# dronefreak/CABiNet

Hardware: AMD Instinct MI355X
Metric: 1024x1024 images/sec fwd+bwd (CABiNet-MobileNetV3-Large) (higher is better)
Workload: dtype f32; 1 GPU; BASELINE configs[2]: CABiNet-MobileNetV3-Large, 8x3x1024x1024 synthetic 8-class per GPU, fwd + 2x OhemCE + bwd + grad all-reduce + SGD step, HIP CAB/FFM kernels, fp32, random-init (model seed 0, gamma=0.5); per_gpu_batch=8, global_batch=8, n_classes=8, parallelism=dp1, miopen_find_mode=FAST

## Files before the change

### cabinet_amd/csrc/conv3x3_s2.hip

```cpp
#include "common.hpp"
#include "slab_sum.hpp"

namespace cabinet {

struct C3Shape {
    int B, H, W, Ho, Wo;
};

static C3Shape c3_shape(int B, int H, int W) { return C3Shape{B, H, W, (H - 1) / 2 + 1, (W - 1) / 2 + 1}; }

constexpr int CW_C = 64;
constexpr int CW_TW = 32;
constexpr int CW_IW = 2 * CW_TW + 1;
constexpr int CW_XP = 3 * CW_IW;
constexpr int CW_DLD = CW_TW + 1;
constexpr int CW_SLAB = CW_C * CW_C * 9;
constexpr int CW_TARGET_WG = 512;
constexpr int CW_MIN_ROWS = 4;

struct C3Plan {
    int tiles_x, strips, rows_per;
};

static C3Plan cw_plan(const C3Shape& s) {
    C3Plan p;
    p.tiles_x = ceil_div(s.Wo, CW_TW);
    const long per = (long)s.B * p.tiles_x;
    long strips = CW_TARGET_WG / per;
    const int cap = ceil_div(s.Ho, CW_MIN_ROWS);
    if (strips > cap) strips = cap;
    if (strips < 1) strips = 1;
    p.rows_per = ceil_div(s.Ho, (int)strips);
    p.strips = ceil_div(s.Ho, p.rows_per);
    return p;
}

__global__ __launch_bounds__(256, 2) void conv3x3s2_wgrad64_kernel(const float* __restrict__ dy, const float* __restrict__ x,
                                                                 C3Shape s, int tiles_x, int strips, int rows_per,
                                                                 float* __restrict__ slabs) {
    extern __shared__ __attribute__((aligned(16))) float smem[];
    float* xs = smem;
    float* dys = xs + CW_C * CW_XP;
    const int tid = threadIdx.x, wave = tid >> 6, lane = tid & 63, li = lane & 31, h = lane >> 5;
    int bi = blockIdx.x;
    const int tx = bi % tiles_x;
    bi /= tiles_x;
    const int strip = bi % strips, b = bi / strips;
    const int oy_begin = strip * rows_per, oy_end = min(s.Ho, oy_begin + rows_per);
    const int ox0 = tx * CW_TW, ix0 = 2 * ox0 - 1;
    const int ch = wave & 1, cj = wave >> 1;

    f32x16 acc[9];
#pragma unroll
    for (int t = 0; t < 9; ++t)
#pragma unroll
        for (int r = 0; r < 16; ++r) acc[t][r] = 0.f;

    const float* xb = x + (size_t)b * CW_C * s.H * s.W;
    const float* dyb = dy + (size_t)b * CW_C * s.Ho * s.Wo;
    const float* arow = dys + (32 * ch + li) * CW_DLD + h;
    const float* brow = xs + (32 * cj + li) * CW_XP + 2 * h;
    for (int oy = oy_begin; oy < oy_end; ++oy) {
        const int iy0 = 2 * oy - 1;
        __syncthreads();
        for (int i = tid; i < CW_C * CW_XP; i += 256) {
            const int ci = i / CW_XP, r = i - ci * CW_XP, yy = r / CW_IW, xx = r - yy * CW_IW;
            const int iy = iy0 + yy, ix = ix0 + xx;
            xs[i] = (iy >= 0 && iy < s.H && ix >= 0 && ix < s.W) ? xb[((size_t)ci * s.H + iy) * s.W + ix] : 0.f;
        }
        for (int i = tid; i < CW_C * CW_TW; i += 256) {
            const int co = i >> 5, c = i & 31, ox = ox0 + c;
            dys[co * CW_DLD + c] = ox < s.Wo ? dyb[((size_t)co * s.Ho + oy) * s.Wo + ox] : 0.f;
        }
        __syncthreads();
#pragma unroll
        for (int c0 = 0; c0 < CW_TW; c0 += 2) {
            const float a = arow[c0];
#pragma unroll
            for (int ky = 0; ky < 3; ++ky)
#pragma unroll
                for (int kx = 0; kx < 3; ++kx)
                    acc[3 * ky + kx] = mfma32(a, brow[ky * CW_IW + 2 * c0 + kx], acc[3 * ky + kx]);
        }
    }
    float* slab = slabs + (size_t)blockIdx.x * CW_SLAB;
#pragma unroll
    for (int r = 0; r < 16; ++r) {
        const int co = 32 * ch + acc_row(r) + 4 * h, ci = 32 * cj + li;
        float* p = slab + (co * CW_C + ci) * 9;
#pragma unroll
        for (int t = 0; t < 9; ++t) p[t] = acc[t][r];
    }
}

constexpr int CF_CI = 3, CF_CO = 16, CF_KK = CF_CI * 9;
constexpr int CF_TH = 4, CF_TW = 32;
constexpr int CF_IH = 2 * CF_TH + 1, CF_IW = 2 * CF_TW + 1;
constexpr int CF_PATCH = CF_CI * CF_IH * CF_IW;
constexpr int CF_DLD = CF_TH * CF_TW + 1;
constexpr int CF_SLAB = CF_CO * CF_KK;

__global__ __launch_bounds__(256) void conv3x3s2_wgrad_3_16_kernel(const float* __restrict__ dy, const float* __restrict__ x,
                                                                  C3Shape s, int tiles_x, float* __restrict__ slabs) {
    __shared__ __attribute__((aligned(16))) float dys[32 * CF_DLD];
    __shared__ float xs[CF_PATCH];
    __shared__ float red[4][CF_CO][32];
    const int tid = threadIdx.x, wave = tid >> 6, lane = tid & 63, li = lane & 31, h = lane >> 5;
    const int strips_y = (s.Ho + CF_TH - 1) / CF_TH;
    const int b = blockIdx.x / strips_y, oy0 = (blockIdx.x - b * strips_y) * CF_TH;
    const int kk = li < CF_KK ? li : 0;
    const int ko = ((kk / 9) * CF_IH + (kk % 9) / 3) * CF_IW + kk % 3;
    f32x16 acc;
#pragma unroll
    for (int r = 0; r < 16; ++r) acc[r] = 0.f;
    for (int i = tid; i < 16 * CF_DLD; i += 256) dys[16 * CF_DLD + i] = 0.f;
    const float* xb = x + (size_t)b * CF_CI * s.H * s.W;
    const float* dyb = dy + (size_t)b * CF_CO * s.Ho * s.Wo;
    const int iy0 = 2 * oy0 - 1;
    for (int t = 0; t < tiles_x; ++t) {
        const int ox0 = t * CF_TW, ix0 = 2 * ox0 - 1;
        __syncthreads();
        for (int i = tid; i < CF_PATCH; i += 256) {
            const int ci = i / (CF_IH * CF_IW), r = i - ci * CF_IH * CF_IW, yy = r / CF_IW, xx = r - yy * CF_IW;
            const int iy = iy0 + yy, ix = ix0 + xx;
            xs[i] = (iy >= 0 && iy < s.H && ix >= 0 && ix < s.W) ? xb[((size_t)ci * s.H + iy) * s.W + ix] : 0.f;
        }
        for (int i = tid; i < CF_CO * CF_TH * CF_TW; i += 256) {
            const int co = i / (CF_TH * CF_TW), p = i - co * (CF_TH * CF_TW), r = p / CF_TW, c = p - r * CF_TW;
            const int oy = oy0 + r, ox = ox0 + c;
            dys[co * CF_DLD + p] = (oy < s.Ho && ox < s.Wo) ? dyb[((size_t)co * s.Ho + oy) * s.Wo + ox] : 0.f;
        }
        __syncthreads();
        const float* drow = dys + li * CF_DLD + 32 * wave + h;
        const float* prow = xs + ko + 2 * wave * CF_IW + 2 * h;
#pragma unroll
        for (int c0 = 0; c0 < 32; c0 += 2) acc = mfma32(drow[c0], prow[2 * c0], acc);
    }
#pragma unroll
    for (int r = 0; r < 16; ++r) {
        const int co = acc_row(r) + 4 * h;
        if (co < CF_CO) red[wave][co][li] = acc[r];
    }
    __syncthreads();
    float* slab = slabs + (size_t)blockIdx.x * CF_SLAB;
    for (int i = tid; i < CF_SLAB; i += 256) {
        const int co = i / CF_KK, k = i - co * CF_KK;
        slab[i] = ((red[0][co][k] + red[1][co][k]) + red[2][co][k]) + red[3][co][k];
    }
}

typedef float f32x4v __attribute__((ext_vector_type(4)));
__device__ __forceinline__ f32x4v mfma16(float a, float b, f32x4v c) { return __builtin_amdgcn_mfma_f32_16x16x4f32(a, b, c, 0, 0, 0); }

constexpr int CD_NT = 64;
constexpr int CD_RP = 80;
constexpr int CD_SLOTS = 3;
constexpr int CD_CP = CD_SLOTS * CD_RP;
constexpr int CD_PR = CW_C / 4;

__device__ __forceinline__ float cd_ld(const float* base, unsigned byte_off) {
    return *reinterpret_cast<const float*>(reinterpret_cast<const char*>(base) + byte_off);
}

__host__ __device__ constexpr int cd_par(int k) { return k == 1 ? 0 : 1; }
__host__ __device__ constexpr int cd_shift(int k) { return k == 0 ? 1 : 0; }

__global__ __launch_bounds__(256, 2) void conv3x3s2_dgrad64_kernel(const float* __restrict__ dy, const float* __restrict__ w,
                                                                 C3Shape s, int tiles_n, int strips, int rows_per,
                                                                 float* __restrict__ dx) {
    __shared__ __attribute__((aligned(16))) float dys[CW_C * CD_CP];
    const int tid = threadIdx.x, wave = __builtin_amdgcn_readfirstlane(tid >> 6), lane = tid & 63, lc = lane & 15, lk = lane >> 4;
    int bi = blockIdx.x;
    const int tn = bi % tiles_n;
    bi /= tiles_n;
    const int strip = bi % strips, b = bi / strips;
    const int m_begin = strip * rows_per, m_end = min(s.Ho, m_begin + rows_per);
    const int n0 = tn * CD_NT;
    const int ci0 = 16 * wave;

    float wr[9][16];
#pragma unroll
    for (int t = 0; t < 9; ++t)
#pragma unroll
        for (int ks = 0; ks < 16; ++ks) wr[t][ks] = w[((4 * ks + lk) * CW_C + ci0 + lc) * 9 + t];

    const float* dyb = dy + (size_t)b * CW_C * s.Ho * s.Wo;
    float* dxb = dx + ((size_t)b * CW_C + ci0 + 4 * lk) * s.H * s.W;
    const float* brow = dys + lk * CD_CP + lc;
    const bool pair_ok = (s.W & 1) == 0;
    const unsigned colo = (unsigned)min(n0 + lane, s.Wo - 1) * 4u;
    const bool col_ok = n0 + lane < s.Wo, halo_ok = n0 + CD_NT < s.Wo;
    float pp[CD_PR + 1];
    auto request = [&](int r) {
        const int oy = min(r, s.Ho - 1);
#pragma unroll
        for (int j = 0; j < CD_PR; ++j) pp[j] = cd_ld(dyb + ((size_t)(CD_PR * wave + j) * s.Ho + oy) * s.Wo, colo);
        int te = tid;
        asm volatile("" : "+v"(te));
        pp[CD_PR] = dyb[((size_t)min(te, CW_C - 1) * s.Ho + oy) * s.Wo + min(n0 + CD_NT, s.Wo - 1)];
    };
    auto commit = [&](int r, int slot) {
        const bool row_ok = r < s.Ho;
        float* d = dys + slot * CD_RP;
#pragma unroll
        for (int j = 0; j < CD_PR; ++j) d[(CD_PR * wave + j) * CD_CP + lane] = (row_ok && col_ok) ? pp[j] : 0.f;
        if (tid < CW_C) d[tid * CD_CP + CD_NT] = (row_ok && halo_ok) ? pp[CD_PR] : 0.f;
    };
    request(m_begin);
    commit(m_begin, 0);
    request(m_begin + 1);
    int s0 = 0;
    for (int m = m_begin; m < m_end; ++m) {
        const int s1 = s0 == CD_SLOTS - 1 ? 0 : s0 + 1;
        commit(m + 1, s1);
        __syncthreads();
        if (m + 1 < m_end) request(m + 2);
        const float* bp0 = brow + s0 * CD_RP;
        const float* bp1 = brow + s1 * CD_RP;
        s0 = s1;
#pragma unroll 1
        for (int ng = 0; ng < CD_NT / 16 && n0 + 16 * ng < s.Wo; ++ng) {
            f32x4v acc[2][2];
#pragma unroll
            for (int i = 0; i < 2; ++i)
#pragma unroll
                for (int j = 0; j < 2; ++j) acc[i][j] = f32x4v{0.f, 0.f, 0.f, 0.f};
            float bv[2][8];
            auto read_half = [&](int g, float* v) {
                const int t = g / 2;
                const float* bt = (cd_shift(t / 3) ? bp1 : bp0) + 16 * ng + cd_shift(t % 3);
#pragma unroll
                for (int i = 0; i < 8; ++i) v[i] = bt[4 * (8 * (g % 2) + i) * CD_CP];
            };
            read_half(0, bv[0]);
            f32x4v p0, p1;
#pragma unroll
            for (int g = 0; g < 18; ++g) {
                const int t = g / 2, k8 = 8 * (g % 2);
                if (g + 1 < 18) read_half(g + 1, bv[(g + 1) & 1]);
                if (g % 2 == 0) p0 = p1 = f32x4v{0.f, 0.f, 0.f, 0.f};
#pragma unroll
                for (int i = 0; i < 8; i += 2) {
                    p0 = mfma16(wr[t][k8 + i], bv[g & 1][i], p0);
                    p1 = mfma16(wr[t][k8 + i + 1], bv[g & 1][i + 1], p1);
                }
                if (g % 2 == 1) acc[cd_par(t / 3)][cd_par(t % 3)] += p0 + p1;
                __builtin_amdgcn_sched_barrier(0);
            }
            const int ix = 2 * (n0 + 16 * ng + lc);
#pragma unroll
            for (int rp = 0; rp < 2; ++rp) {
                const int iy = 2 * m + rp;
                if (iy < s.H && ix < s.W) {
#pragma unroll
                    for (int r = 0; r < 4; ++r) {
                        float* p = dxb + ((size_t)r * s.H + iy) * s.W + ix;
                        if (pair_ok) {
                            *reinterpret_cast<f32x2*>(p) = f32x2{acc[rp][0][r], acc[rp][1][r]};
                        } else {
                            p[0] = acc[rp][0][r];
                            if (ix + 1 < s.W) p[1] = acc[rp][1][r];
                        }
                    }
                }
            }
        }
    }
}

bool conv3x3s2_supported(int Ci, int Co) { return (Ci == CW_C && Co == CW_C) || (Ci == CF_CI && Co == CF_CO); }

static C3Plan cd_plan(const C3Shape& s) {
    C3Plan p;
    p.tiles_x = ceil_div(s.Wo, CD_NT);
    const long per = (long)s.B * p.tiles_x;
    long strips = CW_TARGET_WG / per;
    if (strips > s.Ho) strips = s.Ho;
    if (strips < 1) strips = 1;
    p.rows_per = ceil_div(s.Ho, (int)strips);
    p.strips = ceil_div(s.Ho, p.rows_per);
    return p;
}

long long conv3x3s2_dgrad_workgroups(int B, int H, int W) {
    const C3Shape s = c3_shape(B, H, W);
    const long long per = (long long)B * ceil_div(s.Wo, CD_NT);
    if (per > (1ll << 30)) return per;
    const C3Plan p = cd_plan(s);
    return per * p.strips;
}

hipError_t conv3x3s2_dgrad_run(const float* dy, const float* w, int B, int H, int W, float* dx, hipStream_t stream) {
    const C3Shape s = c3_shape(B, H, W);
    const C3Plan p = cd_plan(s);
    hipLaunchKernelGGL(conv3x3s2_dgrad64_kernel, dim3(B * p.tiles_x * p.strips), dim3(256), 0, stream, dy, w, s, p.tiles_x,
                       p.strips, p.rows_per, dx);
    return hipGetLastError();
}

long long conv3x3s2_wgrad_slabs(int B, int Ci, int H, int W) {
    const C3Shape s = c3_shape(B, H, W);
    if (Ci == CF_CI) return (long long)B * ceil_div(s.Ho, CF_TH);
    const long long tiles_x = ceil_div(s.Wo, CW_TW);
    if ((long long)B * tiles_x > (1ll << 30)) return (long long)B * tiles_x;
    const C3Plan p = cw_plan(s);
    return (long long)B * p.tiles_x * p.strips;
}

size_t conv3x3s2_wgrad_workspace(int B, int Ci, int H, int W) {
    return align_up((size_t)conv3x3s2_wgrad_slabs(B, Ci, H, W) * (Ci == CF_CI ? CF_SLAB : CW_SLAB) * sizeof(float), 256);
}

hipError_t conv3x3s2_wgrad_run(const float* dy, const float* x, int B, int Ci, int H, int W, float* dw, void* ws,
                               hipStream_t stream) {
    const C3Shape s = c3_shape(B, H, W);
    float* slabs = static_cast<float*>(ws);
    const int nslab = (int)conv3x3s2_wgrad_slabs(B, Ci, H, W);
    if (Ci == CF_CI) {
        hipLaunchKernelGGL(conv3x3s2_wgrad_3_16_kernel, dim3(nslab), dim3(256), 0, stream, dy, x, s, ceil_div(s.Wo, CF_TW),
                           slabs);
    } else {
        const C3Plan p = cw_plan(s);
        const size_t lds = (size_t)(CW_C * CW_XP + CW_C * CW_DLD) * sizeof(float);
        static lds_attr_mask mask{0};
        if (hipError_t e = ensure_dynamic_lds(reinterpret_cast<const void*>(conv3x3s2_wgrad64_kernel), lds, mask); e != hipSuccess)
            return e;
        hipLaunchKernelGGL(conv3x3s2_wgrad64_kernel, dim3(nslab), dim3(256), lds, stream, dy, x, s, p.tiles_x, p.strips,
                           p.rows_per, slabs);
    }
    hipError_t e = hipGetLastError();
    if (e != hipSuccess) return e;
    slab_sum_launch(slabs, nslab, Ci == CF_CI ? CF_SLAB : CW_SLAB, dw, stream);
    return hipGetLastError();
}

}
```

### cabinet_amd/functional.py

```python

from __future__ import annotations

import ctypes as _ct

import torch
import torch.nn.functional as F

from . import _lib


def _ptr(t):
    return t.data_ptr() if t is not None else None


def _stream_handle(device):
    return torch.cuda.current_stream(device).cuda_stream


def _workspace(nbytes, device):
    if nbytes == 0:
        return None, 0
    ws = torch.empty(nbytes, dtype=torch.uint8, device=device)
    return ws, nbytes

# ... 1347 lines not shown
        with torch.cuda.device(dev):
            rc = lib.cabinet_se_act_bwd_dx(_ptr(g), _ptr(z), _ptr(mean), _ptr(invstd), _ptr(bn_w), _ptr(bn_b), _ptr(gate), _ptr(ds_p),
                                           _ptr(coef), B, C, P, fn_ctx.act, _ptr(dz), stream)
        _lib.check(rc, "cabinet_se_act_bwd_dx")
        return dz, dweight, dbias, None, None, dw1, db1, dw2, db2, None, None, None, None


def se_tail(z, bn, se, act=None):
    if not z.is_cuda:
        raise RuntimeError("se_tail: device tensors only")
    if act not in _ACT_CODES:
        raise RuntimeError(f"se_tail: unknown activation {act!r}")
    fc1, fc2 = se.fc[0], se.fc[2]
    training, momentum = _bn_step(bn)
    return _SeTail.apply(z, bn.weight, bn.bias, bn.running_mean, bn.running_var, fc1.weight, fc1.bias, fc2.weight, fc2.bias,
                         _ACT_CODES[act], training, momentum, bn.eps)




class _BnActDwConv(torch.autograd.Function):
    @staticmethod
    @torch.amp.custom_fwd(device_type="cuda", cast_inputs=torch.float32)
    def forward(fn_ctx, z, bn_w, bn_b, run_mean, run_var, conv_w, act, stride, training, momentum, eps):
        lib = _lib.load()
        z, bn_w, bn_b, cw = _f32c(z), _f32c(bn_w), _f32c(bn_b), _f32c(conv_w)
        B, C, H, W = z.shape
        K = cw.shape[-1]
        Ho, Wo = (H + 2 * (K // 2) - K) // stride + 1, (W + 2 * (K // 2) - K) // stride + 1
        y = torch.empty((B, C, Ho, Wo), dtype=torch.float32, device=z.device)
        mean = torch.empty(C, dtype=torch.float32, device=z.device)
        invstd = torch.empty(C, dtype=torch.float32, device=z.device)
        ws, nbytes = _workspace(lib.cabinet_bn_dwconv_fwd_workspace_bytes(B, C, H, W), z.device)
        with torch.cuda.device(z.device):
            rc = lib.cabinet_bn_dwconv_fwd(_ptr(z), _ptr(bn_w), _ptr(bn_b), _ptr(run_mean), _ptr(run_var), _ptr(cw), B, C,
                                           H, W, K, stride, act, int(training), float(momentum), float(eps), _ptr(y),
                                           _ptr(mean), _ptr(invstd), _ptr(ws), nbytes, _stream_handle(z.device))
        _lib.check(rc, "cabinet_bn_dwconv_fwd")
        fn_ctx.save_for_backward(z, bn_w, bn_b, cw, mean, invstd)
        fn_ctx.meta = (act, stride, bool(training))
        return y

    @staticmethod
    @torch.amp.custom_bwd(device_type="cuda")
    def backward(fn_ctx, g):
        lib = _lib.load()
        z, bn_w, bn_b, cw, mean, invstd = fn_ctx.saved_tensors
        act, stride, training = fn_ctx.meta
        g = _f32c(g)
        B, C, H, W = z.shape
        K = cw.shape[-1]
        dz, dbw, dbb, dcw = torch.empty_like(z), torch.empty_like(bn_w), torch.empty_like(bn_b), torch.empty_like(cw)
        ws, nbytes = _workspace(lib.cabinet_bn_dwconv_bwd_workspace_bytes(B, C, H, W, K, stride), z.device)
        with torch.cuda.device(z.device):
            rc = lib.cabinet_bn_dwconv_bwd(_ptr(g), _ptr(z), _ptr(bn_w), _ptr(bn_b), _ptr(mean), _ptr(invstd), _ptr(cw), B,
                                           C, H, W, K, stride, act, int(training), _ptr(dz), _ptr(dbw), _ptr(dbb),
                                           _ptr(dcw), _ptr(ws), nbytes, _stream_handle(z.device))
        _lib.check(rc, "cabinet_bn_dwconv_bwd")
        return dz, dbw, dbb, None, None, dcw, None, None, None, None, None


def bn_act_dwconv(z, bn, act, conv):
    if not z.is_cuda:
        raise RuntimeError("bn_act_dwconv: device tensors only")
    if act not in _ACT_CODES:
        raise RuntimeError(f"bn_act_dwconv: unknown activation {act!r}")
    training, momentum = _bn_step(bn)
    return _BnActDwConv.apply(z, bn.weight, bn.bias, bn.running_mean, bn.running_var, conv.weight, _ACT_CODES[act],
                              conv.stride[0], training, momentum, bn.eps)




def stem_conv_supported(conv):
    return (conv.in_channels == 3 and conv.out_channels == 64 and conv.kernel_size == (7, 7) and conv.stride == (2, 2)
            and conv.padding == (3, 3) and conv.dilation == (1, 1) and conv.groups == 1 and conv.bias is None
            and conv.padding_mode == "zeros")


class _StemConv(torch.autograd.Function):
    @staticmethod
    @torch.amp.custom_fwd(device_type="cuda", cast_inputs=torch.float32)
    def forward(fn_ctx, x, weight):
        lib = _lib.load()
        x, w = _f32c(x), _f32c(weight)
        B, _, H, W = x.shape
        y = torch.empty((B, 64, (H - 1) // 2 + 1, (W - 1) // 2 + 1), dtype=torch.float32, device=x.device)
        with torch.cuda.device(x.device):
            rc = lib.cabinet_stem_conv_fwd(_ptr(x), _ptr(w), B, H, W, _ptr(y), _stream_handle(x.device))
        _lib.check(rc, "cabinet_stem_conv_fwd")
        fn_ctx.save_for_backward(x, w)
        return y

    @staticmethod
    @torch.amp.custom_bwd(device_type="cuda")
    def backward(fn_ctx, g):
        lib = _lib.load()
        x, w = fn_ctx.saved_tensors
        g = _f32c(g)
        B, _, H, W = x.shape
        dx = None
        if fn_ctx.needs_input_grad[0]:
            dx = torch.ops.aten.convolution_backward(g, x, w, None, [2, 2], [3, 3], [1, 1], False, [0, 0], 1,
                                                     [True, False, False])[0]
        dw = torch.empty_like(w)
        ws, nbytes = _workspace(lib.cabinet_stem_conv_wrw_workspace_bytes(B, H, W), x.device)
        with torch.cuda.device(x.device):
            rc = lib.cabinet_stem_conv_wrw(_ptr(g), _ptr(x), B, H, W, _ptr(dw), _ptr(ws), nbytes,
                                           _stream_handle(x.device))
        _lib.check(rc, "cabinet_stem_conv_wrw")
        return dx, dw


def stem_conv(x, conv):
    if not x.is_cuda:
        raise RuntimeError("stem_conv: device tensors only")
    return _StemConv.apply(x, conv.weight)


STEM_BN_FUSED = _os.environ.get("CABINET_STEM_BN_FUSED", "1") != "0"


class _StemConvBnRelu(torch.autograd.Function):

    @staticmethod
    @torch.amp.custom_fwd(device_type="cuda", cast_inputs=torch.float32)
    def forward(fn_ctx, x, weight, bn_weight, bn_bias, run_mean, run_var, training, momentum, eps):
        lib = _lib.load()
        x, w, bn_weight, bn_bias = _f32c(x), _f32c(weight), _f32c(bn_weight), _f32c(bn_bias)
        B, _, H, W = x.shape
        z = torch.empty((B, 64, (H - 1) // 2 + 1, (W - 1) // 2 + 1), dtype=torch.float32, device=x.device)
        y = torch.empty_like(z)
        mean = torch.empty(64, dtype=torch.float32, device=x.device)
        invstd = torch.empty(64, dtype=torch.float32, device=x.device)
        P = z.shape[2] * z.shape[3]
        with torch.cuda.device(x.device):
            rc = lib.cabinet_stem_conv_fwd(_ptr(x), _ptr(w), B, H, W, _ptr(z), _stream_handle(x.device))
            _lib.check(rc, "cabinet_stem_conv_fwd")
            ws, nbytes = _workspace(lib.cabinet_bn_act_workspace_bytes(B, 64, P), x.device)
            rc = lib.cabinet_bn_act_fwd(_ptr(z), _ptr(bn_weight), _ptr(bn_bias), _ptr(run_mean), _ptr(run_var), None, B, 64, P,
                                        _ACT_CODES["relu"], int(training), float(momentum), float(eps), _ptr(y), _ptr(mean),
                                        _ptr(invstd), _ptr(ws), nbytes, _stream_handle(x.device))
            _lib.check(rc, "cabinet_bn_act_fwd")
        fn_ctx.save_for_backward(x, z, w, bn_weight, bn_bias, mean, invstd)
        fn_ctx.training = bool(training)
        return y

    @staticmethod
    @torch.amp.custom_bwd(device_type="cuda")
    def backward(fn_ctx, g):
        lib = _lib.load()
        x, z, w, bn_weight, bn_bias, mean, invstd = fn_ctx.saved_tensors
        g = _f32c(g)
        B, _, H, W = x.shape
        dw, dgam, dbet = torch.empty_like(w), torch.empty_like(bn_weight), torch.empty_like(bn_bias)
        ws, nbytes = _workspace(lib.cabinet_stem_conv_bn_bwd_workspace_bytes(B, H, W), x.device)
        with torch.cuda.device(x.device):
            rc = lib.cabinet_stem_conv_bn_bwd(_ptr(g), _ptr(z), _ptr(x), _ptr(bn_weight), _ptr(bn_bias), _ptr(mean), _ptr(invstd),
                                              B, H, W, int(fn_ctx.training), _ptr(dw), _ptr(dgam), _ptr(dbet), _ptr(ws), nbytes,
                                              _stream_handle(x.device))
        _lib.check(rc, "cabinet_stem_conv_bn_bwd")
        return None, dw, dgam, dbet, None, None, None, None, None


def stem_conv_bn_relu(x, conv, bn):
    if not x.is_cuda:
        raise RuntimeError("stem_conv_bn_relu: device tensors only")
    if x.requires_grad:
        raise RuntimeError("stem_conv_bn_relu: the image gets no gradient here; use bn_act(stem_conv(...))")
    training, momentum = _bn_step(bn)
    return _StemConvBnRelu.apply(x, conv.weight, bn.weight, bn.bias, bn.running_mean, bn.running_var, training, momentum, bn.eps)




def pwconv_supported(conv, x):
    if not (conv.kernel_size == (1, 1) and conv.stride == (1, 1) and conv.padding == (0, 0) and conv.groups == 1
            and conv.bias is None and conv.dilation == (1, 1)):
        return False
    P = x.shape[2] * x.shape[3]
    return (P >= 65536 and conv.in_channels <= 96 and conv.out_channels <= 96
            and bool(_lib.load().cabinet_pwconv_supported(conv.in_channels, conv.out_channels, P)))


class _PwConv(torch.autograd.Function):
    @staticmethod
    @torch.amp.custom_fwd(device_type="cuda", cast_inputs=torch.float32)
    def forward(fn_ctx, x, weight):
        lib = _lib.load()
        x = _f32c(x)
        Co, Ci = weight.shape[0], weight.shape[1]
        w2 = _f32c(weight).view(Co, Ci)
        B, P = x.shape[0], x.shape[2] * x.shape[3]
        y = torch.empty((B, Co) + tuple(x.shape[2:]), dtype=torch.float32, device=x.device)
        with torch.cuda.device(x.device):
            rc = lib.cabinet_pwconv_fwd(_ptr(x), _ptr(w2), B, Ci, Co, P, _ptr(y), _stream_handle(x.device))
        _lib.check(rc, "cabinet_pwconv_fwd")
        fn_ctx.save_for_backward(x, w2)
        fn_ctx.w_shape = weight.shape
        return y

    @staticmethod
    @torch.amp.custom_bwd(device_type="cuda")
    def backward(fn_ctx, g):
        lib = _lib.load()
        x, w2 = fn_ctx.saved_tensors
        g = _f32c(g)
        Co, Ci = w2.shape
        B, P = x.shape[0], x.shape[2] * x.shape[3]
        dx = torch.empty_like(x) if fn_ctx.needs_input_grad[0] else None
        dw = torch.empty_like(w2) if fn_ctx.needs_input_grad[1] else None
        ws, nbytes = _workspace(lib.cabinet_pwconv_bwd_workspace_bytes(B, Ci, Co, P), x.device)
        with torch.cuda.device(x.device):
            rc = lib.cabinet_pwconv_bwd(_ptr(g), _ptr(x), _ptr(w2), B, Ci, Co, P, _ptr(dx), _ptr(dw), _ptr(ws), nbytes,
                                        _stream_handle(x.device))
        _lib.check(rc, "cabinet_pwconv_bwd")
        return dx, (dw.view(fn_ctx.w_shape) if dw is not None else None)


def pwconv(x, conv):
    if not x.is_cuda:
        raise RuntimeError("pwconv: device tensors only")
    return _PwConv.apply(x, conv.weight)




PWCONV_WIDE_ENABLED = _os.environ.get("CABINET_PWCONV_WIDE", "1") != "0"


def pwconv_wide_supported(conv, x):
    if not (PWCONV_WIDE_ENABLED and isinstance(conv, torch.nn.Conv2d) and x.is_cuda and x.dim() == 4):
        return False
    if not (conv.kernel_size == (1, 1) and conv.stride == (1, 1) and conv.padding == (0, 0) and conv.groups == 1
            and conv.bias is None and conv.dilation == (1, 1)):
        return False
    if not (torch.is_grad_enabled() and conv.weight.requires_grad) or torch.is_autocast_enabled():
        return False
    if x.dtype != torch.float32 or conv.weight.dtype != torch.float32 or x.shape[0] < 1 or x.shape[2] * x.shape[3] < 1:
        return False
    return bool(_lib.load().cabinet_pwconv_wide_supported(conv.in_channels, conv.out_channels, x.shape[2] * x.shape[3]))


class _PwConvWide(torch.autograd.Function):

    @staticmethod
    def forward(fn_ctx, x, weight):
        x = x.contiguous()
        y = F.conv2d(x, weight)
        fn_ctx.save_for_backward(x, weight)
        return y

    @staticmethod
    def backward(fn_ctx, g):
        x, w = fn_ctx.saved_tensors
        g = g.contiguous()
        dx = None
        if fn_ctx.needs_input_grad[0]:
            dx = torch.ops.aten.convolution_backward(g, x, w, None, [1, 1], [0, 0], [1, 1], False, [0, 0], 1,
                                                     [True, False, False])[0]
        dw = None
        if fn_ctx.needs_input_grad[1]:
            lib = _lib.load()
            xc, gc = _f32c(x), _f32c(g)
            Co, Ci = w.shape[0], w.shape[1]
            B, P = xc.shape[0], xc.shape[2] * xc.shape[3]
            dw = torch.empty((Co, Ci, 1, 1), dtype=torch.float32, device=x.device)
            ws, nbytes = _workspace(lib.cabinet_pwconv_wide_wgrad_workspace_bytes(B, Ci, Co, P), x.device)
            with torch.cuda.device(x.device):
                rc = lib.cabinet_pwconv_wide_wgrad(_ptr(gc), _ptr(xc), B, Ci, Co, P, _ptr(dw), _ptr(ws), nbytes,
                                                   _stream_handle(x.device))
            _lib.check(rc, "cabinet_pwconv_wide_wgrad")
        return dx, dw


def pwconv_wide(x, conv):
    if not x.is_cuda:
        raise RuntimeError("pwconv_wide: device tensors only")
    return _PwConvWide.apply(x, conv.weight)




CONV3X3S2_ENABLED = _os.environ.get("CABINET_CONV3X3S2", "1") != "0"


def conv3x3s2_supported(conv, x):
    if not (CONV3X3S2_ENABLED and isinstance(conv, torch.nn.Conv2d) and x.is_cuda and x.dim() == 4):
        return False
    if not (conv.kernel_size == (3, 3) and conv.stride == (2, 2) and conv.padding == (1, 1) and conv.groups == 1
            and conv.bias is None and conv.dilation == (1, 1) and conv.padding_mode == "zeros"):
        return False
    if not (torch.is_grad_enabled() and conv.weight.requires_grad) or torch.is_autocast_enabled():
        return False
    if x.dtype != torch.float32 or conv.weight.dtype != torch.float32 or x.shape[0] < 1 or x.shape[2] * x.shape[3] < 1:
        return False
    return x.shape[1] == conv.in_channels and bool(_lib.load().cabinet_conv3x3s2_supported(conv.in_channels, conv.out_channels))


def _conv3x3s2_native_wgrad(Ci, B, H):
    return Ci == 3 and B * (((H - 1) // 2 + 1 + 3) // 4) >= 1024


class _Conv3x3S2(torch.autograd.Function):

    @staticmethod
    def forward(fn_ctx, x, weight):
        x = x.contiguous()
        y = F.conv2d(x, weight, None, 2, 1)
        fn_ctx.save_for_backward(x, weight)
        return y

    @staticmethod
    def backward(fn_ctx, g):
        x, w = fn_ctx.saved_tensors
        g = g.contiguous()
        lib = _lib.load()
        xc, gc = _f32c(x), _f32c(g)
        Co, Ci = w.shape[0], w.shape[1]
        B, H, W = xc.shape[0], xc.shape[2], xc.shape[3]
        cb = torch.ops.aten.convolution_backward
        dx = None
        if fn_ctx.needs_input_grad[0] and Ci == 64:
            dx = torch.empty_like(xc)
            with torch.cuda.device(x.device):
                rc = lib.cabinet_conv3x3s2_dgrad(_ptr(gc), _ptr(_f32c(w)), B, Ci, Co, H, W, _ptr(dx), _stream_handle(x.device))
            _lib.check(rc, "cabinet_conv3x3s2_dgrad")
        elif fn_ctx.needs_input_grad[0]:
            dx = cb(g, x, w, None, [2, 2], [1, 1], [1, 1], False, [0, 0], 1, [True, False, False])[0]
        dw = None
        if fn_ctx.needs_input_grad[1] and _conv3x3s2_native_wgrad(Ci, B, H):
            dw = torch.empty((Co, Ci, 3, 3), dtype=torch.float32, device=x.device)
            ws, nbytes = _workspace(lib.cabinet_conv3x3s2_wgrad_workspace_bytes(B, Ci, Co, H, W), x.device)
            with torch.cuda.device(x.device):
                rc = lib.cabinet_conv3x3s2_wgrad(_ptr(gc), _ptr(xc), B, Ci, Co, H, W, _ptr(dw), _ptr(ws), nbytes,
                                                 _stream_handle(x.device))
            _lib.check(rc, "cabinet_conv3x3s2_wgrad")
        elif fn_ctx.needs_input_grad[1]:
            dw = cb(g, x, w, None, [2, 2], [1, 1], [1, 1], False, [0, 0], 1, [False, True, False])[1]
        return dx, dw


class Conv2dS2(torch.nn.Conv2d):

    def _conv_forward(self, input, weight, bias):
        if bias is None and conv3x3s2_supported(self, input):
            return _Conv3x3S2.apply(input, weight)
        return super()._conv_forward(input, weight, bias)




def eval_chip_accum_supported(logits, chip_size, flip=False):
    if not (logits.is_cuda and logits.dim() == 4 and _lib.available()):
        return False
    _, C, hl, wl = logits.shape
    return bool(_lib.load().cabinet_eval_chip_accum_supported(C, hl, wl, int(chip_size[0]), int(chip_size[1]), int(bool(flip))))


def eval_chip_accum(dst, logits, logits_flipped, chip_size, origin, rcp_y=None, rcp_x=None):
    lib = _lib.load()
    if not (dst.is_cuda and dst.dtype == torch.float32 and dst.is_contiguous()):
        raise RuntimeError("eval_chip_accum: dst must be a dense fp32 device tensor")
    a = _f32c(logits)
    b = _f32c(logits_flipped) if logits_flipped is not None else None
    if b is not None and b.shape != a.shape:
        raise RuntimeError("eval_chip_accum: the flipped chip's logits must have the shape of the chip's")
    N, C, hl, wl = a.shape
    if dst.shape[:2] != (N, C):
        raise RuntimeError(f"eval_chip_accum: dst {tuple(dst.shape)} does not match logits {tuple(a.shape)}")
    FH, FW = dst.shape[2:]
    ry = _f32c(rcp_y) if rcp_y is not None else None
    rx = _f32c(rcp_x) if rcp_x is not None else None
    if (ry is not None and ry.numel() != FH) or (rx is not None and rx.numel() != FW):
        raise RuntimeError("eval_chip_accum: rcp_y / rcp_x must have one entry per row / column of dst")
    dev = dst.device
    with torch.cuda.device(dev):
        rc = lib.cabinet_eval_chip_accum(_ptr(a), _ptr(b), N, C, hl, wl, int(chip_size[0]), int(chip_size[1]), _ptr(dst), FH, FW,
                                         int(origin[0]), int(origin[1]), _ptr(ry), _ptr(rx), _stream_handle(dev))
    _lib.check(rc, "cabinet_eval_chip_accum")
    return dst


def eval_scale_merge_supported(total):
    return bool(total.is_cuda and total.dim() == 4 and _lib.available() and total.shape[0] * total.shape[1] <= 65535
                and total.shape[2] <= 65535)


def eval_scale_merge(total, prob, crop=None):
    lib = _lib.load()
    if not (total.is_cuda and total.dtype == torch.float32 and total.is_contiguous()):
        raise RuntimeError("eval_scale_merge: total must be a dense fp32 device tensor")
    prob = _f32c(prob)
    N, C, H, W = total.shape
    if prob.shape[:2] != (N, C):
        raise RuntimeError(f"eval_scale_merge: prob {tuple(prob.shape)} does not match total {tuple(total.shape)}")
    FH, FW = prob.shape[2:]
    hst, hed, wst, wed = crop if crop is not None else (0, FH, 0, FW)
    dev = total.device
    with torch.cuda.device(dev):
        rc = lib.cabinet_eval_scale_merge(_ptr(prob), N, C, FH, FW, int(hst), int(hed), int(wst), int(wed), _ptr(total), H, W,
                                          _stream_handle(dev))
    _lib.check(rc, "cabinet_eval_scale_merge")
    return total


def eval_argmax_hist_supported(total):
    return bool(total.is_cuda and total.dim() == 4 and _lib.available() and total.shape[1] <= 32)


def eval_argmax_hist(total, labels, hist, ignore_label, want_pred=False):
    lib = _lib.load()
    if not (total.is_cuda and total.dtype == torch.float32 and total.is_contiguous()):
        raise RuntimeError("eval_argmax_hist: total must be a dense fp32 device tensor")
    N, C, H, W = total.shape
    if labels.dtype != torch.int64 or tuple(labels.shape) != (N, H, W) or labels.device != total.device:
        raise RuntimeError("eval_argmax_hist: labels must be (N, H, W) int64 on total's device")
    if hist.dtype != torch.int64 or tuple(hist.shape) != (C, C) or not hist.is_contiguous() or hist.device != total.device:
        raise RuntimeError("eval_argmax_hist: hist must be a dense (C, C) int64 tensor on total's device")
    labels = _aligned(labels)
    pred = torch.empty((N, H, W), dtype=torch.uint8, device=total.device) if want_pred else None
    dev = total.device
    with torch.cuda.device(dev):
        rc = lib.cabinet_eval_argmax_hist(_ptr(total), _ptr(labels), N, C, H, W, int(ignore_label), _ptr(hist), _ptr(pred),
                                          _stream_handle(dev))
    _lib.check(rc, "cabinet_eval_argmax_hist")
    return pred




def _u8_out(out, shape, device, what):
    if out is None:
        return torch.empty(shape, dtype=torch.uint8, device=device)
    if not (out.dtype == torch.uint8 and out.device == device and tuple(out.shape) == tuple(shape) and out.is_contiguous()):
        raise RuntimeError(f"{what}: out must be a dense uint8 tensor of shape {tuple(shape)} on the input's device")
    return out


def predict_up_argmax_supported(logits, size):
    if not (logits.is_cuda and logits.dim() == 4 and _lib.available()):
        return False
    N, C, hl, wl = logits.shape
    return bool(N <= 65535 and _lib.load().cabinet_predict_up_argmax_supported(C, hl, wl, int(size[0]), int(size[1])))


def predict_up_argmax(logits, size, out=None):
    lib = _lib.load()
    if not (logits.is_cuda and logits.dim() == 4):
        raise RuntimeError("predict_up_argmax: logits must be a (N, C, h, w) device tensor")
    a = _f32c(logits)
    N, C, hl, wl = a.shape
    H, W = int(size[0]), int(size[1])
    labels = _u8_out(out, (N, H, W), a.device, "predict_up_argmax")
    dev = a.device
    with torch.cuda.device(dev):
        rc = lib.cabinet_predict_up_argmax(_ptr(a), N, C, hl, wl, H, W, _ptr(labels), _stream_handle(dev))
    _lib.check(rc, "cabinet_predict_up_argmax")
    return labels


def predict_argmax_supported(total):
    return bool(total.is_cuda and total.dim() == 4 and _lib.available() and total.shape[1] <= 32 and total.shape[0] <= 65535)


def predict_argmax(total, out=None):
    lib = _lib.load()
    if not (total.is_cuda and total.dim() == 4):
        raise RuntimeError("predict_argmax: total must be a (N, C, H, W) device tensor")
    t = _f32c(total)
    N, C, H, W = t.shape
    labels = _u8_out(out, (N, H, W), t.device, "predict_argmax")
    dev = t.device
    with torch.cuda.device(dev):
        rc = lib.cabinet_predict_argmax(_ptr(t), N, C, H, W, _ptr(labels), _stream_handle(dev))
    _lib.check(rc, "cabinet_predict_argmax")
    return labels


def predict_render(labels, image, palette, mean=(0.485, 0.456, 0.406), std=(0.229, 0.224, 0.225), alpha=0.6,
                   want_input=True, want_overlay=True, out=None):
    lib = _lib.load()
    if not (labels.is_cuda and labels.dtype == torch.uint8 and labels.dim() == 3 and labels.is_contiguous()):
        raise RuntimeError("predict_render: labels must be a dense (N, H, W) uint8 device tensor")
    N, H, W = labels.shape
    dev = labels.device
    if not (palette.dtype == torch.uint8 and palette.dim() == 2 and palette.shape[1] == 3 and palette.device == dev
            and 1 <= palette.shape[0] <= 256):
        raise RuntimeError("predict_render: palette must be a (n_colors <= 256, 3) uint8 tensor on labels' device")
    palette = palette.contiguous()
    img = None
    if image is not None:
        if tuple(image.shape) != (N, 3, H, W) or image.device != dev:
            raise RuntimeError(f"predict_render: image {tuple(image.shape)} does not match labels {tuple(labels.shape)}")
        img = _f32c(image)
    want_input, want_overlay = bool(want_input and img is not None), bool(want_overlay and img is not None)
    out = out or {}
    res = {"pred": _u8_out(out.get("pred"), (N, H, W, 3), dev, "predict_render")}
    if want_input:
        res["input"] = _u8_out(out.get("input"), (N, H, W, 3), dev, "predict_render")
    if want_overlay:
        res["overlay"] = _u8_out(out.get("overlay"), (N, H, W, 3), dev, "predict_render")
    m3, s3 = (_ct.c_float * 3)(*[float(v) for v in mean]), (_ct.c_float * 3)(*[float(v) for v in std])
    with torch.cuda.device(dev):
        rc = lib.cabinet_predict_render(_ptr(labels), _ptr(img if (want_input or want_overlay) else None), _ptr(palette),
                                        int(palette.shape[0]), _ct.addressof(m3), _ct.addressof(s3), float(alpha), N, H, W,
                                        _ptr(res["pred"]), _ptr(res.get("input")), _ptr(res.get("overlay")), _stream_handle(dev))
    _lib.check(rc, "cabinet_predict_render")
    return res
```

Measured before the change: 389.7 images/s.

## Pipeline 64-channel stride-2 conv wgrad with rolling input rows and enable it

Rewrites the 64-channel 3x3 stride-2 weight-gradient kernel so that input rows sit in a three-slot rolling LDS buffer. Each output row now loads only the two new input rows, and those loads are issued into registers before the MFMA loop and committed to LDS afterwards, so global latency overlaps compute and redundant row reloads go away. The Python dispatch now routes Ci==64 layers to this native kernel when the grid is large enough, behind an env flag. Before this, those layers fell back to aten convolution_backward. The cost is more register pressure and extra barriers per row.

```diff
diff --git a/cabinet_amd/csrc/conv3x3_s2.hip b/cabinet_amd/csrc/conv3x3_s2.hip
--- a/cabinet_amd/csrc/conv3x3_s2.hip
+++ b/cabinet_amd/csrc/conv3x3_s2.hip
@@ -35,13 +35,19 @@
     return p;
 }
 
+__device__ __forceinline__ float cd_ld(const float* base, unsigned byte_off) {
+    return *reinterpret_cast<const float*>(reinterpret_cast<const char*>(base) + byte_off);
+}
+
+constexpr int CW_PR = CW_C / 4;
+
 __global__ __launch_bounds__(256, 2) void conv3x3s2_wgrad64_kernel(const float* __restrict__ dy, const float* __restrict__ x,
                                                                  C3Shape s, int tiles_x, int strips, int rows_per,
                                                                  float* __restrict__ slabs) {
     extern __shared__ __attribute__((aligned(16))) float smem[];
     float* xs = smem;
     float* dys = xs + CW_C * CW_XP;
-    const int tid = threadIdx.x, wave = tid >> 6, lane = tid & 63, li = lane & 31, h = lane >> 5;
+    const int tid = threadIdx.x, wave = __builtin_amdgcn_readfirstlane(tid >> 6), lane = tid & 63, li = lane & 31, h = lane >> 5;
     int bi = blockIdx.x;
     const int tx = bi % tiles_x;
     bi /= tiles_x;
@@ -60,28 +66,70 @@
     const float* dyb = dy + (size_t)b * CW_C * s.Ho * s.Wo;
     const float* arow = dys + (32 * ch + li) * CW_DLD + h;
     const float* brow = xs + (32 * cj + li) * CW_XP + 2 * h;
+    const unsigned colo = (unsigned)min(2 * ox0 + lane, s.W - 1) * 4u;
+    const bool col_ok = 2 * ox0 + lane < s.W, halo_ok = ix0 >= 0, dcol_ok = ox0 + li < s.Wo;
+    const int hrow = tid >> 6, hch = tid & 63;
+    const float* dyl = dyb + (size_t)h * s.Ho * s.Wo + min(ox0 + li, s.Wo - 1);
+    float xr[2 * CW_PR], xh, dr[CW_PR / 2];
+    auto request = [&](int nr, int iya, int iyb, bool with_dy, int oy) {
+        const int ya = min(max(iya, 0), s.H - 1), yb = min(max(iyb, 0), s.H - 1);
+#pragma unroll
+        for (int j = 0; j < CW_PR; ++j) xr[j] = cd_ld(xb + ((size_t)(CW_PR * wave + j) * s.H + ya) * s.W, colo);
+        if (nr == 2) {
+#pragma unroll
+            for (int j = 0; j < CW_PR; ++j) xr[CW_PR + j] = cd_ld(xb + ((size_t)(CW_PR * wave + j) * s.H + yb) * s.W, colo);
+        }
+        xh = xb[((size_t)hch * s.H + (hrow == 0 ? ya : yb)) * s.W + max(ix0, 0)];
+        if (with_dy) {
+#pragma unroll
+            for (int j = 0; j < CW_PR / 2; ++j) dr[j] = dyl[((size_t)(CW_PR * wave + 2 * j) * s.Ho + oy) * s.Wo];
+        }
+    };
+    auto commit = [&](int nr, int iya, int iyb, int sa, int sb, bool with_dy) {
+        const bool oka = iya >= 0 && iya < s.H, okb = iyb >= 0 && iyb < s.H;
+        float* d = xs + CW_PR * wave * CW_XP + 1 + lane;
+#pragma unroll
+        for (int j = 0; j < CW_PR; ++j) d[j * CW_XP + sa * CW_IW] = (oka && col_ok) ? xr[j] : 0.f;
+        if (nr == 2) {
+#pragma unroll
+            for (int j = 0; j < CW_PR; ++j) d[j * CW_XP + sb * CW_IW] = (okb && col_ok) ? xr[CW_PR + j] : 0.f;
+        }
+        if (hrow < nr) xs[hch * CW_XP + (hrow == 0 ? sa : sb) * CW_IW] = ((hrow == 0 ? oka : okb) && halo_ok) ? xh : 0.f;
+        if (with_dy) {
+#pragma unroll
+            for (int j = 0; j < CW_PR / 2; ++j) dys[(CW_PR * wave + 2 * j + h) * CW_DLD + li] = dcol_ok ? dr[j] : 0.f;
+        }
+    };
+    const int iy_begin = 2 * oy_begin - 1;
+    request(2, iy_begin, iy_begin + 1, true, oy_begin);
+    commit(2, iy_begin, iy_begin + 1, 0, 1, true);
+    request(1, iy_begin + 2, iy_begin + 2, false, 0);
+    commit(1, iy_begin + 2, iy_begin + 2, 2, 2, false);
+    __syncthreads();
+    int s0 = 0;
     for (int oy = oy_begin; oy < oy_end; ++oy) {
-        const int iy0 = 2 * oy - 1;
-        __syncthreads();
-        for (int i = tid; i < CW_C * CW_XP; i += 256) {
-            const int ci = i / CW_XP, r = i - ci * CW_XP, yy = r / CW_IW, xx = r - yy * CW_IW;
-            const int iy = iy0 + yy, ix = ix0 + xx;
-            xs[i] = (iy >= 0 && iy < s.H && ix >= 0 && ix < s.W) ? xb[((size_t)ci * s.H + iy) * s.W + ix] : 0.f;
-        }
-        for (int i = tid; i < CW_C * CW_TW; i += 256) {
-            const int co = i >> 5, c = i & 31, ox = ox0 + c;
-            dys[co * CW_DLD + c] = ox < s.Wo ? dyb[((size_t)co * s.Ho + oy) * s.Wo + ox] : 0.f;
-        }
-        __syncthreads();
+        const int s1 = s0 == 2 ? 0 : s0 + 1, s2 = s1 == 2 ? 0 : s1 + 1;
+        const bool more = oy + 1 < oy_end;
+        if (more) request(2, 2 * oy + 2, 2 * oy + 3, true, oy + 1);
+        const float* b0 = brow + s0 * CW_IW;
+        const float* b1 = brow + s1 * CW_IW;
+        const float* b2 = brow + s2 * CW_IW;
 #pragma unroll
         for (int c0 = 0; c0 < CW_TW; c0 += 2) {
             const float a = arow[c0];
 #pragma unroll
-            for (int ky = 0; ky < 3; ++ky)
-#pragma unroll
-                for (int kx = 0; kx < 3; ++kx)
-                    acc[3 * ky + kx] = mfma32(a, brow[ky * CW_IW + 2 * c0 + kx], acc[3 * ky + kx]);
-        }
+            for (int kx = 0; kx < 3; ++kx) acc[kx] = mfma32(a, b0[2 * c0 + kx], acc[kx]);
+#pragma unroll
+            for (int kx = 0; kx < 3; ++kx) acc[3 + kx] = mfma32(a, b1[2 * c0 + kx], acc[3 + kx]);
+#pragma unroll
+            for (int kx = 0; kx < 3; ++kx) acc[6 + kx] = mfma32(a, b2[2 * c0 + kx], acc[6 + kx]);
+        }
+        if (more) {
+            __syncthreads();
+            commit(2, 2 * oy + 2, 2 * oy + 3, s0, s1, true);
+            __syncthreads();
+        }
+        s0 = s2;
     }
     float* slab = slabs + (size_t)blockIdx.x * CW_SLAB;
 #pragma unroll
@@ -157,10 +205,6 @@
 constexpr int CD_SLOTS = 3;
 constexpr int CD_CP = CD_SLOTS * CD_RP;
 constexpr int CD_PR = CW_C / 4;
-
-__device__ __forceinline__ float cd_ld(const float* base, unsigned byte_off) {
-    return *reinterpret_cast<const float*>(reinterpret_cast<const char*>(base) + byte_off);
-}
 
 __host__ __device__ constexpr int cd_par(int k) { return k == 1 ? 0 : 1; }
 __host__ __device__ constexpr int cd_shift(int k) { return k == 0 ? 1 : 0; }
diff --git a/cabinet_amd/functional.py b/cabinet_amd/functional.py
--- a/cabinet_amd/functional.py
+++ b/cabinet_amd/functional.py
@@ -1673,6 +1673,26 @@
     return Ci == 3 and B * (((H - 1) // 2 + 1 + 3) // 4) >= 1024
 
 
+CONV3X3S2_WGRAD64_ENABLED = _os.environ.get("CABINET_CONV3X3S2_WGRAD64", "1") != "0"
+_CW_MIN_WORKGROUPS = 256
+_CW_MIN_ROWS = 4
+
+
+def _conv3x3s2_wgrad64_plan(B, H, W):
+    Ho, Wo = (H - 1) // 2 + 1, (W - 1) // 2 + 1
+    tiles = -(-Wo // 32)
+    strips = max(1, min(512 // (B * tiles), -(-Ho // 4)))
+    rows_per = -(-Ho // strips)
+    return B * tiles * -(-Ho // rows_per), rows_per
+
+
+def _conv3x3s2_native_wgrad64(B, H, W):
+    if not CONV3X3S2_WGRAD64_ENABLED:
+        return False
+    workgroups, rows_per = _conv3x3s2_wgrad64_plan(B, H, W)
+    return workgroups >= _CW_MIN_WORKGROUPS and rows_per >= _CW_MIN_ROWS
+
+
 class _Conv3x3S2(torch.autograd.Function):
 
     @staticmethod
@@ -1700,7 +1720,8 @@
         elif fn_ctx.needs_input_grad[0]:
             dx = cb(g, x, w, None, [2, 2], [1, 1], [1, 1], False, [0, 0], 1, [True, False, False])[0]
         dw = None
-        if fn_ctx.needs_input_grad[1] and _conv3x3s2_native_wgrad(Ci, B, H):
+        native_dw = _conv3x3s2_native_wgrad64(B, H, W) if Ci == 64 else _conv3x3s2_native_wgrad(Ci, B, H)
+        if fn_ctx.needs_input_grad[1] and native_dw:
             dw = torch.empty((Co, Ci, 3, 3), dtype=torch.float32, device=x.device)
             ws, nbytes = _workspace(lib.cabinet_conv3x3s2_wgrad_workspace_bytes(B, Ci, Co, H, W), x.device)
             with torch.cuda.device(x.device):
```

After: 396.4 images/s, median of 6. 1.7% higher.
